# RL-VIG/LibContinual

Measured on AMD Instinct MI355X. Metric: images/sec/node (task-0 epoch), CIFAR-100 B50-5x10, higher is better.
Workload: dtype bf16; 1 GPU; lwf_resnet18_b50_task0; method=LWF, backbone=resnet18, per_gpu_batch=256, global_batch=256, image=3x32x32, parallelism=dp1, optimizer=fused SGD

## Files before the change

### libcontinual_amd/csrc/conv4.hip

```cpp
#include <stdlib.h>

#include "common.h"

namespace {

int g_force4[4] = {0, 0, 0, 0};
int g_enable4 = -1, g_debug4 = 0;
unsigned long long* g_trace4 = nullptr;

typedef __attribute__((ext_vector_type(16))) float f32x16;
typedef __attribute__((ext_vector_type(4))) unsigned u32x4;
typedef __attribute__((address_space(1))) const void gvoid_t;
typedef __attribute__((address_space(3))) void lvoid_t;

struct Conv4Params {
    const bf16_t* src;
    const bf16_t* wt;
    bf16_t* dst;
    float* stats;
    double* stat_acc;
    int stat_rep;
    const bf16_t* bn_z;
    const bf16_t* bn_y;
    const float* bn_mean;
    const float* bn_invstd;
    double* bn_acc;
    int bn_rep;
    int H, W, Cs, Cd, M, accumulate;
    int wshift, hshift;
    int np;
    int patch_bytes;
    int n_ntiles, nt_shift, n_items;
    int cpg;
    unsigned long long* trace;
    int debug;
};

template <int MODE>
__device__ __forceinline__ unsigned tap_mask4(int g, const Conv4Params& p) {
    int w, h;
    if (p.wshift >= 0 && p.hshift >= 0) { w = g & (p.W - 1); h = (g >> p.wshift) & (p.H - 1); }
    else { w = g % p.W; h = (g / p.W) % p.H; }
    constexpr unsigned UP = MODE == 0 ? 0x007u : 0x1c0u, DOWN = MODE == 0 ? 0x1c0u : 0x007u;
    constexpr unsigned LEFT = MODE == 0 ? 0x049u : 0x124u, RIGHT = MODE == 0 ? 0x124u : 0x049u;
    unsigned m = 0x1ffu;
    if (h == 0) m &= ~UP;
    if (h == p.H - 1) m &= ~DOWN;
    if (w == 0) m &= ~LEFT;
    if (w == p.W - 1) m &= ~RIGHT;
    return m;
}

#ifdef CLHIP_ABLATION
#define DBG(p) ((p).debug)
#define STAMP() do { if (p.trace && blockIdx.x == 0 && lane == 0 && (wave & 3) == 0 && nstamp < 256) p.trace[(wave >> 2) * 256 + nstamp++] = __builtin_amdgcn_s_memtime(); } while (0)
#else
#define STAMP() do { } while (0)
#define DBG(p) 0
#endif

template <int N> __device__ __forceinline__ void wait_vm() { __builtin_amdgcn_s_waitcnt((N & 15) | 0x70 | 0xF00 | ((N >> 4) << 14)); }
__device__ __forceinline__ void wait_lds() { __builtin_amdgcn_s_waitcnt(0xC07F); }
__device__ __forceinline__ void wg_barrier(bool skip = false) {
    wait_lds();
    if (!skip) __builtin_amdgcn_s_barrier();
    asm volatile("" ::: "memory");
}

template <int WM, int WN, int KG, int CK, int WMAX, int MODE>
__global__ __launch_bounds__(WM * WN * KG * 64, 2) void conv4_kernel(const Conv4Params p) {
    constexpr int BM = WM * 64, BN = WN * 64, NWG = WM * WN, NTG = NWG * 64;
    constexpr int NST = 3;
    constexpr int PP = CK * 2 + 16;
    constexpr int KS = CK / 16;
    constexpr int WROW = CK * 2;
    constexpr int SPR = WROW / 16;
    constexpr int RPI = 64 / SPR;
    constexpr int SLAB = BN * WROW;
    constexpr int WINST = (BN / RPI) / NWG;
    static_assert((BN / RPI) % NWG == 0 && WINST >= 1, "ring rows must divide among the waves of a group");
    constexpr int SPP = PP / 16;
    constexpr int ZBYTES = 512;
    constexpr int PINST = ((((BM + 2 * WMAX + 2) * PP + 255) / 256 * 256 + ZBYTES) / 1024 + 1 + NWG - 1) / NWG;
    constexpr int PL_TAP = 2;
    constexpr bool SETPRIO = false;
    constexpr bool STAG = NWG * KG == 8;

    extern __shared__ __attribute__((aligned(16))) char smem[];
    const int tid = threadIdx.x, lane = tid & 63;
    const int wave = __builtin_amdgcn_readfirstlane(tid >> 6);
    const int grp = wave / NWG, wv = wave % NWG;
    int nstamp = 0; (void)nstamp;
    const int wm = wv / WN, wn = wv % WN;
    const int l31 = lane & 31, kh = lane >> 5;
    const int W = p.W, Cs = p.Cs, halo = W + 1;
    const int K9 = 9 * Cs;

    char* patch_g = smem + grp * 2 * p.patch_bytes;
    char* ring0 = smem + KG * 2 * p.patch_bytes;
    char* ring_g = ring0 + grp * SLAB;
    constexpr int XR_BYTES = KG > 1 ? (KG - 1) * NWG * 64 * 64 * 4 : 0;
    const int ring_end = KG * 2 * p.patch_bytes + NST * KG * SLAB;
    float* red = reinterpret_cast<float*>(smem + (ring_end > XR_BYTES ? ring_end : XR_BYTES));

    int xaddr[2];
#pragma unroll
    for (int i = 0; i < 2; ++i) xaddr[i] = (wm * 64 + i * 32 + l31 + halo) * PP + kh * 16;
    const int zoff = (p.np * PP + 255) / 256 * 256;
    int waddr[2][KS];
#pragma unroll
    for (int j = 0; j < 2; ++j) {
        const int o = wn * 64 + j * 32 + l31;
        const int swz = CK == 64 ? ((o >> 1) & 7) : ((o >> 2) & 3);
#pragma unroll
        for (int ks = 0; ks < KS; ++ks) waddr[j][ks] = o * WROW + (((2 * ks + kh) ^ swz) << 4);
    }
    unsigned dma_lane[WINST];
#pragma unroll
    for (int i = 0; i < WINST; ++i) {
        const int row = (wv * WINST + i) * RPI + lane / SPR;
        const int slot = lane % SPR;
        const int swz = CK == 64 ? ((row >> 1) & 7) : ((row >> 2) & 3);
        dma_lane[i] = (unsigned)((row * K9 + (slot ^ swz) * 8) * 2);
    }
    const char* wbase = reinterpret_cast<const char*>(p.wt);
    auto dma = [&](int item, int cc, int tap, int stage) {
        const int n0 = (item & (p.n_ntiles - 1)) * BN;
        const size_t uni = ((size_t)n0 * K9 + (size_t)tap * Cs + (size_t)(grp * p.cpg + cc) * CK) * 2;
        const char* g = wbase + uni;
        char* l = ring_g + stage * (KG * SLAB) + wv * (WINST * 1024);
        if (DBG(p) & 2) return;
#if defined(__HIP_DEVICE_COMPILE__)
#pragma unroll
        for (int i = 0; i < WINST; ++i)
            __builtin_amdgcn_global_load_lds((gvoid_t*)(g + dma_lane[i]), (lvoid_t*)(l + i * 1024), 16, 0, 0);
#else
        (void)g; (void)l;
#endif
    };

    const __amdgpu_buffer_rsrc_t srs = __builtin_amdgcn_make_buffer_rsrc(const_cast<bf16_t*>(p.src), 0, p.M * Cs * 2, 0x00020000);
    constexpr int OOB = 0x40000000;
    int prel[PINST];
#pragma unroll
    for (int i = 0; i < PINST; ++i) {
        const int slot = (wv * PINST + i) * 64 + lane;
        const int q = slot / SPP, sub = slot - q * SPP;
        prel[i] = (q < p.np && sub < SPP - 1) ? q * (Cs * 2) + sub * 16 : OOB;
    }
    auto pdma = [&](int item, int cc, int buf) {
        const int m0 = (item >> p.nt_shift) * BM;
        const int base = (m0 - halo) * (Cs * 2) + (grp * p.cpg + cc) * CK * 2;
        char* l = patch_g + buf * p.patch_bytes + wv * (PINST * 1024);
#if defined(__HIP_DEVICE_COMPILE__)
#pragma unroll
        for (int i = 0; i < PINST; ++i)
            __builtin_amdgcn_raw_ptr_buffer_load_lds(srs, (lvoid_t*)(l + i * 1024), 16, prel[i] + base, 0, 0, 0);
#else
        (void)base; (void)l;
#endif
    };

    const int G = gridDim.x;
    const int nmy = (p.n_items - (int)blockIdx.x + G - 1) / G;
    const int cpg = p.cpg;

    const bool pl_on = !(DBG(p) & 4);
    if (pl_on) pdma(blockIdx.x, 0, 0);
    dma(blockIdx.x, 0, 0, 0);
    dma(blockIdx.x, 0, 1, 1);
    if constexpr (STAG) {
        wait_vm<WINST>();
    } else {
        dma(blockIdx.x, 0, 2, 2);
        wait_vm<2 * WINST>();
    }
    wg_barrier();

    constexpr int UK = STAG ? KS : KS / 2;
    bf16x8_t ax[UK][2], aw[UK][2], bx[UK][2], bw[UK][2];
    int cur = 0;
    for (int k = 0; k < nmy; ++k) {
        const int item = blockIdx.x + k * G;
        const int m0 = (item >> p.nt_shift) * BM, n0 = (item & (p.n_ntiles - 1)) * BN;
        unsigned tmask[2];
#pragma unroll
        for (int i = 0; i < 2; ++i) {
            const int g = m0 + wm * 64 + i * 32 + l31;
            tmask[i] = g < p.M ? tap_mask4<MODE>(g, p) : 0u;
        }
        auto frags = [&](bf16x8_t (&xf)[UK][2], bf16x8_t (&wf)[UK][2], const char* pb, int r, int s, int u) {
            if (DBG(p) & 64) return;
            const char* ws = ring_g + s * (KG * SLAB);
            const int shift = (MODE == 0 ? (r - 1) * W + (s - 1) : (1 - r) * W + (1 - s)) * PP;
            const unsigned bit = 1u << (3 * r + s);
            int xa[2];
#pragma unroll
            for (int i = 0; i < 2; ++i) { const int a = xaddr[i] + shift; xa[i] = (tmask[i] & bit) ? a : zoff + (a & 255); }
#pragma unroll
            for (int q = 0; q < UK; ++q) {
#pragma unroll
                for (int i = 0; i < 2; ++i) xf[q][i] = *reinterpret_cast<const bf16x8_t*>(pb + xa[i] + (u * UK + q) * 32);
#pragma unroll
                for (int j = 0; j < 2; ++j) wf[q][j] = *reinterpret_cast<const bf16x8_t*>(ws + waddr[j][u * UK + q]);
            }
        };
        f32x16 acc[2][2];
#pragma unroll
        for (int j = 0; j < 2; ++j)
#pragma unroll
            for (int i = 0; i < 2; ++i)
#pragma unroll
                for (int r = 0; r < 16; ++r) acc[j][i][r] = 0.f;
        auto mma = [&](const bf16x8_t (&xf)[UK][2], const bf16x8_t (&wf)[UK][2]) {
            if (DBG(p) & 1) {
#pragma unroll
                for (int q = 0; q < UK; ++q)
#pragma unroll
                    for (int j = 0; j < 2; ++j) asm volatile("" ::"v"(xf[q][j]), "v"(wf[q][j]));
                return;
            }
#pragma unroll
            for (int q = 0; q < UK; ++q)
#pragma unroll
                for (int j = 0; j < 2; ++j)
#pragma unroll
                    for (int i = 0; i < 2; ++i) acc[j][i] = __builtin_amdgcn_mfma_f32_32x32x16_bf16(wf[q][j], xf[q][i], acc[j][i], 0, 0, 0);
        };

        if constexpr (STAG) {
            constexpr int NU = KS / UK;
            const bool lag = wave >= 4;
            if (lag) __builtin_amdgcn_s_barrier();
            for (int cc = 0; cc < cpg; ++cc, cur ^= 1) {
                int ncc = cc + 1, nk = k;
                if (ncc == cpg) { ncc = 0; nk = k + 1; }
                const bool nvalid = nk < nmy;
                const int nitem = blockIdx.x + nk * G;
                const char* pb = patch_g + cur * p.patch_bytes;
                const bool pl = nvalid && pl_on;
#pragma unroll 1
                for (int r = 0; r < 3; ++r) {
#pragma unroll
                    for (int s = 0; s < 3; ++s) {
#pragma unroll
                        for (int u = 0; u < NU; ++u) {
                            frags(ax, aw, pb, r, s, u);
                            if (u == 0) {
                                if (s == 0) dma(item, cc, 3 * r + 2, 2);
                                else if (r < 2) dma(item, cc, 3 * (r + 1) + s - 1, s - 1);
                                else if (nvalid) dma(nitem, ncc, s - 1, s - 1);
                                if (s == PL_TAP && r == 0 && pl) pdma(nitem, ncc, cur ^ 1);
                            }
                            STAMP();
                            if (u == NU - 1) {
                                const bool d2 = (s == 0 || r < 2) ? true : nvalid;
                                if (d2) {
                                    if (((s == PL_TAP && r == 0) || (s == 0 && r == 1)) && pl) wait_vm<WINST + PINST>();
                                    else wait_vm<WINST>();
                                } else {
                                    wait_vm<0>();
                                }
                            }
                            __builtin_amdgcn_sched_barrier(0);
                            STAMP();
                            wait_lds();
                            STAMP();
                            __builtin_amdgcn_s_barrier();
                            STAMP();
                            __builtin_amdgcn_sched_barrier(0);
                            if (SETPRIO) __builtin_amdgcn_s_setprio(1);
                            mma(ax, aw);
                            if (SETPRIO) __builtin_amdgcn_s_setprio(0);
                            __builtin_amdgcn_sched_barrier(0);
                            STAMP();
                            __builtin_amdgcn_s_barrier();
                            STAMP();
                        }
                    }
                }
            }
            if (!lag) __builtin_amdgcn_s_barrier();
        } else {
        frags(ax, aw, patch_g + cur * p.patch_bytes, 0, 0, 0);
        for (int cc = 0; cc < cpg; ++cc, cur ^= 1) {
            int ncc = cc + 1, nk = k;
            if (ncc == cpg) { ncc = 0; nk = k + 1; }
            const bool nvalid = nk < nmy;
            const bool last_chunk = ncc == 0;
            const int nitem = blockIdx.x + nk * G;
            const char* pb = patch_g + cur * p.patch_bytes;
            const char* pbn = patch_g + (cur ^ 1) * p.patch_bytes;
#pragma unroll 1
            for (int r = 0; r < 3; ++r) {
#pragma unroll
                for (int s = 0; s < 3; ++s) {
                    wait_lds();
                    frags(bx, bw, pb, r, s, 1);
                    __builtin_amdgcn_sched_barrier(0);
                    mma(ax, aw);
                    __builtin_amdgcn_sched_barrier(0);
                    const bool pl = nvalid && pl_on;
                    if (s == PL_TAP && r == 0 && pl) pdma(nitem, ncc, cur ^ 1);
                    const bool d2 = (r < 2 || s == 0) ? true : nvalid;
                    if (d2) {
                        if (((s == PL_TAP && r == 0) || (s == 0 && r == 1)) && pl) wait_vm<WINST + PINST>();
                        else wait_vm<WINST>();
                    } else {
                        wait_vm<0>();
                    }
                    wg_barrier(DBG(p) & 32);
                    if (r < 2) dma(item, cc, 3 * (r + 1) + s, s);
                    else if (nvalid) dma(nitem, ncc, s, s);
                    if (s < 2) frags(ax, aw, pb, r, s + 1, 0);
                    else if (r < 2) frags(ax, aw, pb, r + 1, 0, 0);
                    else if (!last_chunk) frags(ax, aw, pbn, 0, 0, 0);
                    __builtin_amdgcn_sched_barrier(0);
                    mma(bx, bw);
                    __builtin_amdgcn_sched_barrier(0);
                }
            }
        }

        }

        if constexpr (KG > 1) {
            wait_vm<0>();
            float* xr = reinterpret_cast<float*>(smem);
            if (grp > 0) {
                float* q = xr + ((size_t)((grp - 1) * NWG + wv) * 64) * 64;
#pragma unroll
                for (int j = 0; j < 2; ++j)
#pragma unroll
                    for (int i = 0; i < 2; ++i)
#pragma unroll
                        for (int r4 = 0; r4 < 4; ++r4)
                            *reinterpret_cast<f32x4*>(q + ((j * 2 + i) * 4 + r4) * 256 + lane * 4) =
                                f32x4{acc[j][i][4 * r4], acc[j][i][4 * r4 + 1], acc[j][i][4 * r4 + 2], acc[j][i][4 * r4 + 3]};
            }
            wg_barrier();
            if (grp > 0) return;
#pragma unroll
            for (int g2 = 1; g2 < KG; ++g2) {
                const float* q = xr + ((size_t)((g2 - 1) * NWG + wv) * 64) * 64;
#pragma unroll
                for (int j = 0; j < 2; ++j)
#pragma unroll
                    for (int i = 0; i < 2; ++i)
#pragma unroll
                        for (int r4 = 0; r4 < 4; ++r4) {
                            const f32x4 v = *reinterpret_cast<const f32x4*>(q + ((j * 2 + i) * 4 + r4) * 256 + lane * 4);
                            acc[j][i][4 * r4] += v[0]; acc[j][i][4 * r4 + 1] += v[1]; acc[j][i][4 * r4 + 2] += v[2]; acc[j][i][4 * r4 + 3] += v[3];
                        }
            }
        }

#pragma unroll
        for (int i = 0; i < 2; ++i) {
            const int pix = m0 + wm * 64 + i * 32 + l31;
            const bool pv = pix < p.M;
            bf16_t* drow = p.dst + (size_t)pix * p.Cd + n0 + wn * 64;
#pragma unroll
            for (int j = 0; j < 2; ++j) {
                if (MODE == 1 && p.accumulate && pv) {
#pragma unroll
                    for (int g4 = 0; g4 < 4; ++g4) {
                        const uint2 old = *reinterpret_cast<const uint2*>(drow + j * 32 + g4 * 8 + kh * 4);
                        acc[j][i][4 * g4 + 0] += __uint_as_float(old.x << 16); acc[j][i][4 * g4 + 1] += __uint_as_float(old.x & 0xffff0000u);
                        acc[j][i][4 * g4 + 2] += __uint_as_float(old.y << 16); acc[j][i][4 * g4 + 3] += __uint_as_float(old.y & 0xffff0000u);
                    }
                }
#pragma unroll
                for (int pr = 0; pr < 2; ++pr) {
                    unsigned ax = pack_bf16x2(acc[j][i][8 * pr + 0], acc[j][i][8 * pr + 1]), ay = pack_bf16x2(acc[j][i][8 * pr + 2], acc[j][i][8 * pr + 3]);
                    unsigned bx = pack_bf16x2(acc[j][i][8 * pr + 4], acc[j][i][8 * pr + 5]), by = pack_bf16x2(acc[j][i][8 * pr + 6], acc[j][i][8 * pr + 7]);
                    auto rx = __builtin_amdgcn_permlane32_swap(ax, bx, false, false);
                    auto ry = __builtin_amdgcn_permlane32_swap(ay, by, false, false);
                    if (pv && !(DBG(p) & 8)) *reinterpret_cast<u32x4*>(drow + j * 32 + pr * 16 + kh * 8) = u32x4{rx[0], ry[0], rx[1], ry[1]};
                }
            }
        }
        const bool fwd_stats = MODE == 0 && (p.stats != nullptr || p.stat_acc != nullptr) && !(DBG(p) & 16);
        const bool bwd_sums = MODE == 1 && p.bn_z != nullptr;
        if (fwd_stats || bwd_sums) {
#pragma unroll
            for (int j = 0; j < 2; ++j) {
                float sv[32];
                if (MODE == 0) {
#pragma unroll
                    for (int r = 0; r < 16; ++r) {
                        const float a = acc[j][0][r], b = acc[j][1][r];
                        sv[r] = a + b;
                        sv[16 + r] = fmaf(a, a, b * b);
                    }
                } else {
#pragma unroll
                    for (int r = 0; r < 32; ++r) sv[r] = 0.f;
#pragma unroll
                    for (int i = 0; i < 2; ++i) {
                        const int pix = m0 + wm * 64 + i * 32 + l31;
                        if (pix < p.M) {
                            const size_t row = (size_t)pix * p.Cd + n0 + wn * 64 + j * 32 + kh * 4;
#pragma unroll
                            for (int g4 = 0; g4 < 4; ++g4) {
                                const uint2 zz = *reinterpret_cast<const uint2*>(p.bn_z + row + g4 * 8);
                                uint2 yy = make_uint2(0x3f803f80u, 0x3f803f80u);
                                if (p.bn_y != nullptr) yy = *reinterpret_cast<const uint2*>(p.bn_y + row + g4 * 8);
                                const float z4[4] = {__uint_as_float(zz.x << 16), __uint_as_float(zz.x & 0xffff0000u), __uint_as_float(zz.y << 16), __uint_as_float(zz.y & 0xffff0000u)};
                                const float y4[4] = {__uint_as_float(yy.x << 16), __uint_as_float(yy.x & 0xffff0000u), __uint_as_float(yy.y << 16), __uint_as_float(yy.y & 0xffff0000u)};
#pragma unroll
                                for (int e = 0; e < 4; ++e) {
                                    const float g = y4[e] > 0.f ? acc[j][i][4 * g4 + e] : 0.f;
                                    sv[4 * g4 + e] += g;
                                    sv[16 + 4 * g4 + e] = fmaf(g, z4[e], sv[16 + 4 * g4 + e]);
                                }
                            }
                        }
                    }
                }
                row16_sum_n(sv);
                if ((lane & 15) == 0) {
                    const int rh = (lane >> 4) & 1;
#pragma unroll
                    for (int which = 0; which < 2; ++which)
#pragma unroll
                        for (int g4 = 0; g4 < 4; ++g4) {
                            const int cc2 = wn * 64 + j * 32 + g4 * 8 + kh * 4;
                            const float* v = sv + which * 16 + g4 * 4;
                            *reinterpret_cast<f32x4*>(red + ((wm * 2 + rh) * 2 + which) * BN + cc2) = f32x4{v[0], v[1], v[2], v[3]};
                        }
                }
            }
            wg_barrier();
            for (int idx = tid; idx < 2 * BN; idx += NTG) {
                const int which = idx / BN, c2 = idx - which * BN;
                float t = 0.f;
#pragma unroll
                for (int w2 = 0; w2 < WM * 2; ++w2) t += red[(w2 * 2 + which) * BN + c2];
                const int mt = item >> p.nt_shift;
                if (MODE == 0) {
                    if (p.stat_acc != nullptr) atomicAdd(p.stat_acc + ((size_t)(mt & (p.stat_rep - 1)) * 2 + which) * p.Cd + n0 + c2, (double)t);
                    else p.stats[((size_t)mt * 2 + which) * p.Cd + n0 + c2] = t;
                } else {
                    if (which == 1) {
                        float sg = 0.f;
#pragma unroll
                        for (int w2 = 0; w2 < WM * 2; ++w2) sg += red[(w2 * 2 + 0) * BN + c2];
                        t = p.bn_invstd[n0 + c2] * (t - p.bn_mean[n0 + c2] * sg);
                    }
                    atomicAdd(p.bn_acc + ((size_t)(mt & (p.bn_rep - 1)) * 2 + which) * p.Cd + n0 + c2, (double)t);
                }
            }
        }
    }
}

struct Cfg4 { int wm, wn, kg, ck; };

template <int WM, int WN, int KG, int CK, int WMAX, int MODE>
int launch4(Conv4Params& p, hipStream_t st) {
    constexpr int BM = WM * 64, BN = WN * 64, PP = CK * 2 + 16, NWG = WM * WN;
    p.np = BM + 2 * p.W + 2;
    p.patch_bytes = (((((BM + 2 * WMAX + 2) * PP + 255) / 256 * 256 + 512) / 1024 + 1 + NWG - 1) / NWG) * NWG * 1024;
    p.n_ntiles = p.Cd / BN;
    p.nt_shift = ilog2_exact(p.n_ntiles);
    const int n_mtiles = (p.M + BM - 1) / BM;
    p.n_items = n_mtiles * p.n_ntiles;
    p.cpg = (p.Cs / CK) / KG;
    size_t lds = (size_t)KG * 2 * p.patch_bytes + (size_t)3 * KG * BN * CK * 2;
    if (KG > 1) { size_t x = (size_t)(KG - 1) * NWG * 64 * 64 * sizeof(float); if (x > lds) lds = x; }
    lds += (size_t)WM * 2 * 2 * BN * sizeof(float);
    if (lds > 160 * 1024) { clhip_set_error("conv4: %zu bytes of LDS", lds); return CLHIP_EINVAL; }
    auto kern = conv4_kernel<WM, WN, KG, CK, WMAX, MODE>;
    static size_t attr = 0;
    if (lds > attr) {
        if (hipFuncSetAttribute(reinterpret_cast<const void*>(kern), hipFuncAttributeMaxDynamicSharedMemorySize, (int)lds) != hipSuccess) {
            clhip_set_error("conv4: cannot reserve %zu bytes of LDS", lds);
            return CLHIP_EHIP;
        }
        attr = lds;
    }
    int per_cu = (int)((160 * 1024) / lds);
    const int wave_cap = 8 / (NWG * KG) > 0 ? 8 / (NWG * KG) : 1;
    if (per_cu > wave_cap) per_cu = wave_cap;
    if (per_cu < 1) per_cu = 1;
    static const int force_grid = clhip_cfg("CONV4_GRID") ? atoi(clhip_cfg("CONV4_GRID")) : 0;
    int grid = 256 * per_cu;
    if (force_grid > 0) grid = force_grid;
    if (KG > 1 || grid > p.n_items) grid = p.n_items;
    hipLaunchKernelGGL(kern, dim3(grid), dim3(NWG * KG * 64), lds, st, p);
    CLHIP_LAUNCH_CHECK();
    return CLHIP_OK;
}

Cfg4 pick4(int M, int Cs, int Cd, int W) {
    static const char* ov = clhip_cfg("CONV4_CFG");
    if (g_force4[0] > 0) return Cfg4{g_force4[0], g_force4[1], g_force4[2], g_force4[3]};
    if (ov) { Cfg4 c{0, 0, 0, 0}; if (sscanf(ov, "%d,%d,%d,%d", &c.wm, &c.wn, &c.kg, &c.ck) == 4) return c; }
    auto tiles = [&](int bm, int bn) { return (int64_t)((M + bm - 1) / bm) * (Cd / bn); };
    if (Cd % 128 == 0 && tiles(256, 128) >= 200) return Cfg4{4, 2, 1, 64};
    if (Cd % 128 == 0 && tiles(128, 128) >= 200 && (Cs / 32) % 2 == 0) return Cfg4{2, 2, 2, 32};
    if (tiles(256, 64) >= 256) return Cfg4{4, 1, 1, 32};
    if (tiles(64, 64) <= 256 && (Cs / 32) % 4 == 0 && W <= 16) return Cfg4{1, 1, 4, 32};
    if (W <= 8 && tiles(128, 64) >= 128 && (Cs / 64) % 2 == 0) return Cfg4{2, 1, 2, 64};
    if ((Cs / 32) % 2 == 0) return Cfg4{2, 1, 2, 32};
    return Cfg4{2, 1, 1, 32};
}

bool cfg_ok(const Cfg4& c, int Cs, int Cd) {
    if (!(c.ck == 32 || c.ck == 64)) return false;
    if (Cs % c.ck || Cd % (c.wn * 64)) return false;
    if ((Cs / c.ck) % c.kg) return false;
    const int nt = Cd / (c.wn * 64);
    return (nt & (nt - 1)) == 0;
}

}

bool clhip_conv4_supported(int N, int H, int W, int Cs, int Cd, int ksize, int stride, int pad, int dtype) {
    static const bool on = clhip_cfg("CONV4") ? atoi(clhip_cfg("CONV4")) != 0 : true;
    if (g_enable4 >= 0 ? g_enable4 == 0 : !on) return false;
    if (!(dtype == CLHIP_BF16 && ksize == 3 && stride == 1 && pad == 1 && (Cs % 64) == 0 && (Cd % 64) == 0 && W <= 32 && W >= 2 && H >= 1)) return false;
    if ((int64_t)N * H * W * (Cs > Cd ? Cs : Cd) * 2 >= ((int64_t)1 << 29)) return false;
    const int nt = Cd / 64;
    return (nt & (nt - 1)) == 0;
}

int clhip_conv4_tiles_m(int M, int Cs, int Cd, int W) { return (M + pick4(M, Cs, Cd, W).wm * 64 - 1) / (pick4(M, Cs, Cd, W).wm * 64); }

int clhip_conv4_launch_bn(const void* src, const void* wt, void* dst, float* stats, double* stat_acc, int stat_rep, int N, int H, int W, int Cs, int Cd,
                          int accumulate, int mode, const void* bn_z, const void* bn_y, const float* bn_mean, const float* bn_invstd, double* bn_acc, int bn_rep,
                          hipStream_t st);

int clhip_conv4_launch(const void* src, const void* wt, void* dst, float* stats, double* stat_acc, int stat_rep, int N, int H, int W, int Cs, int Cd,
                       int accumulate, int mode, hipStream_t st) {
    return clhip_conv4_launch_bn(src, wt, dst, stats, stat_acc, stat_rep, N, H, W, Cs, Cd, accumulate, mode, nullptr, nullptr, nullptr, nullptr, nullptr, 1, st);
}

int clhip_conv4_launch_bn(const void* src, const void* wt, void* dst, float* stats, double* stat_acc, int stat_rep, int N, int H, int W, int Cs, int Cd,
                          int accumulate, int mode, const void* bn_z, const void* bn_y, const float* bn_mean, const float* bn_invstd, double* bn_acc, int bn_rep,
                          hipStream_t st) {
    Conv4Params p;
    p.bn_z = static_cast<const bf16_t*>(bn_z); p.bn_y = static_cast<const bf16_t*>(bn_y); p.bn_mean = bn_mean; p.bn_invstd = bn_invstd;
    p.bn_acc = bn_acc; p.bn_rep = bn_rep > 0 ? bn_rep : 1;
    p.src = static_cast<const bf16_t*>(src); p.wt = static_cast<const bf16_t*>(wt); p.dst = static_cast<bf16_t*>(dst);
    p.stats = stats; p.stat_acc = stat_acc; p.stat_rep = stat_rep > 0 ? stat_rep : 1;
    p.H = H; p.W = W; p.wshift = ilog2_exact(W); p.hshift = ilog2_exact(H); p.Cs = Cs; p.Cd = Cd; p.accumulate = accumulate; p.M = N * H * W;
    p.debug = g_debug4; p.trace = g_trace4;
    Cfg4 c = pick4(p.M, Cs, Cd, W);
    if (!cfg_ok(c, Cs, Cd)) { clhip_set_error("conv4: configuration %d,%d,%d,%d does not fit Cs=%d Cd=%d", c.wm, c.wn, c.kg, c.ck, Cs, Cd); return CLHIP_EINVAL; }
#define L4(a, b, g, k) (W <= 8 ? (mode == 0 ? launch4<a, b, g, k, 8, 0>(p, st) : launch4<a, b, g, k, 8, 1>(p, st)) \
                               : (mode == 0 ? launch4<a, b, g, k, 32, 0>(p, st) : launch4<a, b, g, k, 32, 1>(p, st)))
    const int key = c.wm * 1000 + c.wn * 100 + c.kg * 10 + (c.ck == 64 ? 1 : 0);
    switch (key) {
        case 4110: return L4(4, 1, 1, 32);
        case 4111: return L4(4, 1, 1, 64);
        case 2110: return L4(2, 1, 1, 32);
        case 2111: return L4(2, 1, 1, 64);
        case 2210: return L4(2, 2, 1, 32);
        case 2211: return L4(2, 2, 1, 64);
        case 4210: return L4(4, 2, 1, 32);
        case 4211: return L4(4, 2, 1, 64);
        case 2120: return L4(2, 1, 2, 32);
        case 2121: return L4(2, 1, 2, 64);
        case 1220: return L4(1, 2, 2, 32);
        case 2220: return L4(2, 2, 2, 32);
        case 1140: return L4(1, 1, 4, 32);
        case 1141: return L4(1, 1, 4, 64);
        case 2140: return L4(2, 1, 4, 32);
        case 2141: return L4(2, 1, 4, 64);
        case 1240: return L4(1, 2, 4, 32);
        default: break;
    }
#undef L4
    clhip_set_error("conv4: no kernel for configuration %d,%d,%d,%d", c.wm, c.wn, c.kg, c.ck);
    return CLHIP_EINVAL;
}

void clhip_conv4_set_cfg(int wm, int wn, int kg, int ck) { g_force4[0] = wm; g_force4[1] = wn; g_force4[2] = kg; g_force4[3] = ck; }
void clhip_conv4_enable(int on) { g_enable4 = on; }
void clhip_conv4_set_debug(int bits) { g_debug4 = bits; }
void clhip_conv4_set_trace(unsigned long long* dev_buf) { g_trace4 = dev_buf; }

bool clhip_conv4_in_supported(int N, int H, int W, int Cs, int Cd) { (void)N; (void)H; (void)W; (void)Cs; (void)Cd; return false; }
int clhip_conv4_launch_in(const void* src, const void* wt, void* dst, double* stat_acc, int stat_rep, int N, int H, int W, int Cs, int Cd, const LazyIn* in, hipStream_t st) {
    (void)src; (void)wt; (void)dst; (void)stat_acc; (void)stat_rep; (void)N; (void)H; (void)W; (void)Cs; (void)Cd; (void)in; (void)st;
    clhip_set_error("conv4: lazy inputs are not supported");
    return CLHIP_EINVAL;
}
```

Before: 132,000 images/sec.

## Fuse producer BN+ReLU (and residual) into conv4 input patch loading

Adds a lazy-input path to the implicit-GEMM conv kernel. The producer's batch-norm scale/shift, optional residual add and ReLU are applied to the staged input patch in LDS, the normalized activation and ReLU mask are written out once by the owning tile, and the supported-check is enabled so callers can skip a separate BN/ReLU elementwise pass. This trades an extra global read and write pass for in-kernel ALU work spread across tap iterations, extra LDS, and a halved occupancy bound for some configs.

```diff
diff --git a/libcontinual_amd/csrc/conv4.hip b/libcontinual_amd/csrc/conv4.hip
--- a/libcontinual_amd/csrc/conv4.hip
+++ b/libcontinual_amd/csrc/conv4.hip
@@ -33,6 +33,7 @@
     int n_ntiles, nt_shift, n_items;
     int cpg;
     unsigned long long* trace;
+    LazyIn in;
     int debug;
 };
 
@@ -67,8 +68,10 @@
     asm volatile("" ::: "memory");
 }
 
-template <int WM, int WN, int KG, int CK, int WMAX, int MODE>
-__global__ __launch_bounds__(WM * WN * KG * 64, 2) void conv4_kernel(const Conv4Params p) {
+template <int WM, int WN, int KG, int CK, int WMAX, int MODE, int XF = 0>
+__global__ __launch_bounds__(WM * WN * KG * 64, (XF != 0 && WM * WN * KG == 4) ? 1 : 2) void conv4_kernel(const Conv4Params p) {
+    static_assert(XF == 0 || MODE == 0, "lazy inputs exist in the forward only");
+    static_assert(XF == 0 || WM * WN * KG >= 4, "the coefficient prologue wants 256 threads");
     constexpr int BM = WM * 64, BN = WN * 64, NWG = WM * WN, NTG = NWG * 64;
     constexpr int NST = 3;
     constexpr int PP = CK * 2 + 16;
@@ -102,6 +105,10 @@
     constexpr int XR_BYTES = KG > 1 ? (KG - 1) * NWG * 64 * 64 * 4 : 0;
     const int ring_end = KG * 2 * p.patch_bytes + NST * KG * SLAB;
     float* red = reinterpret_cast<float*>(smem + (ring_end > XR_BYTES ? ring_end : XR_BYTES));
+    constexpr int MPP = CK / 8, MSB = BM * MPP;
+    constexpr int RED_F = (XF != 0 && WM * 2 * 2 * BN < 512) ? 512 : WM * 2 * 2 * BN;
+    float* coefs = red + RED_F;
+    unsigned char* mst_g = reinterpret_cast<unsigned char*>(coefs + 2 * p.Cs) + grp * 2 * MSB;
 
     int xaddr[2];
 #pragma unroll
@@ -161,6 +168,72 @@
 #endif
     };
 
+    uint4 rr[XF == 2 ? PINST : 1];
+    auto res_load = [&](int item, int cc) __attribute__((always_inline)) {
+        if constexpr (XF == 2) {
+            const int g0 = (item >> p.nt_shift) * BM - halo;
+            const bf16_t* rb = p.in.res + (grp * p.cpg + cc) * CK;
+#pragma unroll
+            for (int i = 0; i < PINST; ++i) {
+                const int slot = (wv * PINST + i) * 64 + lane;
+                const int q = slot / SPP, sub = slot - q * SPP, g = g0 + q;
+                rr[i] = make_uint4(0, 0, 0, 0);
+                if (prel[i] != OOB && g >= 0 && g < p.M) rr[i] = *reinterpret_cast<const uint4*>(rb + (size_t)g * Cs + sub * 8);
+            }
+        }
+    };
+    auto xpiece = [&](int i, int item, int cc, int buf) __attribute__((always_inline)) {
+        int ln = lane;
+        asm volatile("" : "+v"(ln));
+        const int slot = (wv * PINST + i) * 64 + ln;
+        const int q = slot / SPP, sub = slot - q * SPP;
+        const int g = (item >> p.nt_shift) * BM - halo + q;
+        if (prel[i] != OOB && g >= 0 && g < p.M) {
+            char* l = patch_g + buf * p.patch_bytes + slot * 16;
+            const int c0 = (grp * p.cpg + cc) * CK + sub * 8;
+            const uint4 v = *reinterpret_cast<const uint4*>(l);
+            float sc[8], sh[8];
+            *reinterpret_cast<f32x4*>(sc) = *reinterpret_cast<const f32x4*>(coefs + c0);
+            *reinterpret_cast<f32x4*>(sc + 4) = *reinterpret_cast<const f32x4*>(coefs + c0 + 4);
+            *reinterpret_cast<f32x4*>(sh) = *reinterpret_cast<const f32x4*>(coefs + Cs + c0);
+            *reinterpret_cast<f32x4*>(sh + 4) = *reinterpret_cast<const f32x4*>(coefs + Cs + c0 + 4);
+            uint4 o;
+            unsigned mk = 0;
+            if constexpr (XF == 2) o = bn_res_relu8_bf16(v, rr[i], sc, sh, mk);
+            else o = bn_relu8_bf16(v, sc, sh);
+            *reinterpret_cast<uint4*>(l) = o;
+            const bool own = q >= halo && q < halo + BM && (item & (p.n_ntiles - 1)) == 0;
+            if (own) {
+                *reinterpret_cast<uint4*>(p.in.y + (size_t)g * Cs + c0) = o;
+                if (XF == 2 && p.in.mask != nullptr) mst_g[buf * MSB + (q - halo) * MPP + sub] = (unsigned char)mk;
+            }
+        }
+    };
+    auto xform = [&](int k, int item, int cc, int buf) __attribute__((always_inline)) {
+        if constexpr (XF != 0) {
+            asm volatile("" ::: "memory");
+#pragma unroll
+            for (int i = 0; i < PINST; ++i)
+                if (k < 0 || (i * 5) / PINST == k) xpiece(i, item, cc, buf);
+        }
+    };
+    auto mask_flush = [&](int item, int cc, int buf) __attribute__((always_inline)) {
+        if constexpr (XF == 2) {
+            if (p.in.mask != nullptr && (item & (p.n_ntiles - 1)) == 0) {
+                const int m0f = (item >> p.nt_shift) * BM;
+                unsigned char* mrow = p.in.mask + ((grp * p.cpg + cc) * CK >> 3);
+                for (int t = wv * 64 + lane; t < BM; t += NTG) {
+                    const int g = m0f + t;
+                    if (g < p.M) {
+                        if constexpr (MPP == 8) *reinterpret_cast<uint2*>(mrow + (size_t)g * (Cs >> 3)) = *reinterpret_cast<const uint2*>(mst_g + buf * MSB + t * 8);
+                        else *reinterpret_cast<unsigned*>(mrow + (size_t)g * (Cs >> 3)) = *reinterpret_cast<const unsigned*>(mst_g + buf * MSB + t * 4);
+                    }
+                }
+            }
+        }
+    };
+    constexpr int XPI = XF == 2 ? PINST : 0;
+
     const int G = gridDim.x;
     const int nmy = (p.n_items - (int)blockIdx.x + G - 1) / G;
     const int cpg = p.cpg;
@@ -169,10 +242,15 @@
     if (pl_on) pdma(blockIdx.x, 0, 0);
     dma(blockIdx.x, 0, 0, 0);
     dma(blockIdx.x, 0, 1, 1);
-    if constexpr (STAG) {
+    if constexpr (!STAG) dma(blockIdx.x, 0, 2, 2);
+    if constexpr (XF != 0) {
+        res_load(blockIdx.x, 0);
+        lazy_in_coefs(p.in, Cs, coefs, reinterpret_cast<double*>(red), blockIdx.x == 0);
+        wait_vm<0>();
+        xform(-1, blockIdx.x, 0, 0);
+    } else if constexpr (STAG) {
         wait_vm<WINST>();
     } else {
-        dma(blockIdx.x, 0, 2, 2);
         wait_vm<2 * WINST>();
     }
     wg_barrier();
@@ -239,6 +317,7 @@
                 const int nitem = blockIdx.x + nk * G;
                 const char* pb = patch_g + cur * p.patch_bytes;
                 const bool pl = nvalid && pl_on;
+                mask_flush(item, cc, cur);
 #pragma unroll 1
                 for (int r = 0; r < 3; ++r) {
 #pragma unroll
@@ -250,16 +329,22 @@
                                 if (s == 0) dma(item, cc, 3 * r + 2, 2);
                                 else if (r < 2) dma(item, cc, 3 * (r + 1) + s - 1, s - 1);
                                 else if (nvalid) dma(nitem, ncc, s - 1, s - 1);
-                                if (s == PL_TAP && r == 0 && pl) pdma(nitem, ncc, cur ^ 1);
+                                if (s == PL_TAP && r == 0 && pl) { pdma(nitem, ncc, cur ^ 1); res_load(nitem, ncc); }
                             }
                             STAMP();
                             if (u == NU - 1) {
                                 const bool d2 = (s == 0 || r < 2) ? true : nvalid;
                                 if (d2) {
-                                    if (((s == PL_TAP && r == 0) || (s == 0 && r == 1)) && pl) wait_vm<WINST + PINST>();
+                                    if (((s == PL_TAP && r == 0) || (s == 0 && r == 1)) && pl) wait_vm<WINST + PINST + XPI>();
                                     else wait_vm<WINST>();
                                 } else {
                                     wait_vm<0>();
+                                }
+                                if constexpr (XF != 0) {
+                                    if (pl) {
+                                        if (r == 1 && s >= 1) xform(s - 1, nitem, ncc, cur ^ 1);
+                                        else if (r == 2) xform(s + 2, nitem, ncc, cur ^ 1);
+                                    }
                                 }
                             }
                             __builtin_amdgcn_sched_barrier(0);
@@ -291,6 +376,7 @@
             const int nitem = blockIdx.x + nk * G;
             const char* pb = patch_g + cur * p.patch_bytes;
             const char* pbn = patch_g + (cur ^ 1) * p.patch_bytes;
+            mask_flush(item, cc, cur);
 #pragma unroll 1
             for (int r = 0; r < 3; ++r) {
 #pragma unroll
@@ -301,13 +387,19 @@
                     mma(ax, aw);
                     __builtin_amdgcn_sched_barrier(0);
                     const bool pl = nvalid && pl_on;
-                    if (s == PL_TAP && r == 0 && pl) pdma(nitem, ncc, cur ^ 1);
+                    if (s == PL_TAP && r == 0 && pl) { pdma(nitem, ncc, cur ^ 1); res_load(nitem, ncc); }
                     const bool d2 = (r < 2 || s == 0) ? true : nvalid;
                     if (d2) {
-                        if (((s == PL_TAP && r == 0) || (s == 0 && r == 1)) && pl) wait_vm<WINST + PINST>();
+                        if (((s == PL_TAP && r == 0) || (s == 0 && r == 1)) && pl) wait_vm<WINST + PINST + XPI>();
                         else wait_vm<WINST>();
                     } else {
                         wait_vm<0>();
+                    }
+                    if constexpr (XF != 0) {
+                        if (pl) {
+                            if (r == 1 && s >= 1) xform(s - 1, nitem, ncc, cur ^ 1);
+                            else if (r == 2) xform(s + 2, nitem, ncc, cur ^ 1);
+                        }
                     }
                     wg_barrier(DBG(p) & 32);
                     if (r < 2) dma(item, cc, 3 * (r + 1) + s, s);
@@ -457,7 +549,7 @@
 
 struct Cfg4 { int wm, wn, kg, ck; };
 
-template <int WM, int WN, int KG, int CK, int WMAX, int MODE>
+template <int WM, int WN, int KG, int CK, int WMAX, int MODE, int XF = 0>
 int launch4(Conv4Params& p, hipStream_t st) {
     constexpr int BM = WM * 64, BN = WN * 64, PP = CK * 2 + 16, NWG = WM * WN;
     p.np = BM + 2 * p.W + 2;
@@ -469,9 +561,10 @@
     p.cpg = (p.Cs / CK) / KG;
     size_t lds = (size_t)KG * 2 * p.patch_bytes + (size_t)3 * KG * BN * CK * 2;
     if (KG > 1) { size_t x = (size_t)(KG - 1) * NWG * 64 * 64 * sizeof(float); if (x > lds) lds = x; }
-    lds += (size_t)WM * 2 * 2 * BN * sizeof(float);
+    lds += (size_t)((XF != 0 && WM * 2 * 2 * BN < 512) ? 512 : WM * 2 * 2 * BN) * sizeof(float);
+    if (XF != 0) lds += (size_t)2 * p.Cs * sizeof(float) + (XF == 2 ? (size_t)KG * 2 * BM * (CK / 8) : 0);
     if (lds > 160 * 1024) { clhip_set_error("conv4: %zu bytes of LDS", lds); return CLHIP_EINVAL; }
-    auto kern = conv4_kernel<WM, WN, KG, CK, WMAX, MODE>;
+    auto kern = conv4_kernel<WM, WN, KG, CK, WMAX, MODE, XF>;
     static size_t attr = 0;
     if (lds > attr) {
         if (hipFuncSetAttribute(reinterpret_cast<const void*>(kern), hipFuncAttributeMaxDynamicSharedMemorySize, (int)lds) != hipSuccess) {
@@ -582,9 +675,34 @@
 void clhip_conv4_set_debug(int bits) { g_debug4 = bits; }
 void clhip_conv4_set_trace(unsigned long long* dev_buf) { g_trace4 = dev_buf; }
 
-bool clhip_conv4_in_supported(int N, int H, int W, int Cs, int Cd) { (void)N; (void)H; (void)W; (void)Cs; (void)Cd; return false; }
+namespace {
+bool in_cfg4(const Cfg4& c) {
+    return (c.wm == 4 && c.wn == 2 && c.kg == 1 && c.ck == 64) || (c.wm == 2 && c.wn == 2 && c.kg == 2 && c.ck == 32) || (c.wm == 2 && c.wn == 1 && c.kg == 2 && c.ck == 64) ||
+           (c.wm == 1 && c.wn == 1 && c.kg == 4 && c.ck == 32);
+}
+}
+
+bool clhip_conv4_in_supported(int N, int H, int W, int Cs, int Cd) {
+    const Cfg4 c = pick4(N * H * W, Cs, Cd, W);
+    return in_cfg4(c) && cfg_ok(c, Cs, Cd) && Cs <= 512;
+}
+
 int clhip_conv4_launch_in(const void* src, const void* wt, void* dst, double* stat_acc, int stat_rep, int N, int H, int W, int Cs, int Cd, const LazyIn* in, hipStream_t st) {
-    (void)src; (void)wt; (void)dst; (void)stat_acc; (void)stat_rep; (void)N; (void)H; (void)W; (void)Cs; (void)Cd; (void)in; (void)st;
-    clhip_set_error("conv4: lazy inputs are not supported");
-    return CLHIP_EINVAL;
-}
+    if (in == nullptr || in->acc == nullptr || in->y == nullptr) { clhip_set_error("conv4: a lazy input needs the producer's sums and an output activation"); return CLHIP_EINVAL; }
+    Conv4Params p;
+    p.bn_z = nullptr; p.bn_y = nullptr; p.bn_mean = nullptr; p.bn_invstd = nullptr; p.bn_acc = nullptr; p.bn_rep = 1;
+    p.src = static_cast<const bf16_t*>(src); p.wt = static_cast<const bf16_t*>(wt); p.dst = static_cast<bf16_t*>(dst);
+    p.stats = nullptr; p.stat_acc = stat_acc; p.stat_rep = stat_rep > 0 ? stat_rep : 1;
+    p.H = H; p.W = W; p.wshift = ilog2_exact(W); p.hshift = ilog2_exact(H); p.Cs = Cs; p.Cd = Cd; p.accumulate = 0; p.M = N * H * W;
+    p.debug = g_debug4; p.trace = g_trace4;
+    p.in = *in;
+    const Cfg4 c = pick4(p.M, Cs, Cd, W);
+    if (!in_cfg4(c) || !cfg_ok(c, Cs, Cd) || Cs > 512) { clhip_set_error("conv4: no lazy-input kernel for configuration %d,%d,%d,%d", c.wm, c.wn, c.kg, c.ck); return CLHIP_EINVAL; }
+#define L4X(a, b, g, k) (W <= 8 ? (in->res != nullptr ? launch4<a, b, g, k, 8, 0, 2>(p, st) : launch4<a, b, g, k, 8, 0, 1>(p, st)) \
+                                : (in->res != nullptr ? launch4<a, b, g, k, 32, 0, 2>(p, st) : launch4<a, b, g, k, 32, 0, 1>(p, st)))
+    if (c.wm == 4) return L4X(4, 2, 1, 64);
+    if (c.wm == 1) return L4X(1, 1, 4, 32);
+    if (c.wn == 2) return L4X(2, 2, 2, 32);
+    return L4X(2, 1, 2, 64);
+#undef L4X
+}
```

New measurement: 131,900 images/sec. Within noise of the previous version (-0.1%).
